# vLAR-group/unMORE

Measured on AMD Instinct MI355X. Metric: images/sec (train fwd+bwd) ObjectnessNet ViT-B/16 384x384, higher is better.
Workload: dtype bf16

## Files before the change

### unmore_amd/csrc/gemm_nt256p.hip

```cpp
#include "umr_common.h"
#include "gemm_epilogue.h"
#include <stdio.h>
#include <stdlib.h>
#include <type_traits>

namespace {

constexpr int BM2 = 256, BN2 = 256, BK2 = 64;
constexpr int ROWB2 = 128;
constexpr int TILE2 = 256 * ROWB2;
constexpr int BUF2 = 2 * TILE2;
constexpr int STG_OFF = 2 * BUF2;
constexpr int STG_BYTES = 32 * 256 * 4;
constexpr int LDS2P = STG_OFF + STG_BYTES;

typedef bf16_t T2;

__device__ __forceinline__ unsigned mul_dgelu_bf16x2(unsigned g, unsigned x) {
    const float lo = __builtin_bit_cast(float, g << 16) * dgelu_sel<bf16_t>(__builtin_bit_cast(float, x << 16));
    const float hi = __builtin_bit_cast(float, g & 0xFFFF0000u) * dgelu_sel<bf16_t>(__builtin_bit_cast(float, x & 0xFFFF0000u));
    typedef __attribute__((ext_vector_type(2))) __bf16 bf16x2;
    bf16x2 r;
    r[0] = (bf16_t)lo; r[1] = (bf16_t)hi;
    return __builtin_bit_cast(unsigned, r);
}

__device__ __forceinline__ unsigned add_bf16x2(unsigned x, unsigned y) {
    const float lo = __builtin_bit_cast(float, x << 16) + __builtin_bit_cast(float, y << 16);
    const float hi = __builtin_bit_cast(float, x & 0xFFFF0000u) + __builtin_bit_cast(float, y & 0xFFFF0000u);
    typedef __attribute__((ext_vector_type(2))) __bf16 bf16x2;
    bf16x2 r;
    r[0] = (bf16_t)lo; r[1] = (bf16_t)hi;
    return __builtin_bit_cast(unsigned, r);
}

__device__ __forceinline__ unsigned pos_mask_bf16x2(unsigned a) {
    typedef __attribute__((ext_vector_type(2))) short s16x2;
    const s16x2 one = {1, 1}, zero = {0, 0};
    s16x2 v = __builtin_bit_cast(s16x2, a);
    v = __builtin_elementwise_min(v, one);
    v = __builtin_elementwise_max(v, zero);
    v = zero - v;
    return __builtin_bit_cast(unsigned, v);
}

template <int CONV, int EPI, int AUXM, bool RED, bool X3 = false, bool P2 = true>
__global__ __launch_bounds__(512, 2) void gemm_nt256p_kernel(const umr_gemm_desc p, int tiles_n, int total_tiles, int stagger, int bm, int npairs = 6,
                                                             int kt_per_arg = 0) {
    const int sp = (X3 && kt_per_arg > 0) ? (int)blockIdx.y : 0;
    static_assert(X3 == (EPI == 5 || EPI == 6), "the plane-pair K loop and the f32 / plane epilogues (EPI 5, 6) go together");
    constexpr bool PH2 = P2;
    static_assert(CONV == 0 || P2, "the conv is instantiated in its two-phase form only");
    extern __shared__ __attribute__((aligned(16))) char smem[];
    constexpr int SZ = 2;
    constexpr unsigned OOB = 0x80000000u;
    const int tid = threadIdx.x, lane = tid & 63;
    const int w = __builtin_amdgcn_readfirstlane(tid >> 6);
    const bool ahead = (stagger != 0) && (w < 4);

    const int G = gridDim.x;
    const int pw = ((G & 7) == 0) ? (int)(blockIdx.x & 7) * (G >> 3) + (int)(blockIdx.x >> 3) : (int)blockIdx.x;
    if (pw >= total_tiles) return;
    const int n_my = (total_tiles - pw + G - 1) / G;

    const int lrow = lane >> 3, lchk = lane & 7;
    const int hw = (CONV != 0) ? p.Ho * p.Wo : 1;
    const int apix = X3 ? 3 * p.Cin : p.Cin;
    unsigned vo[4][2];
    int trow_a[2][2];
    unsigned a_tapmask[2][2];
    unsigned a_eff[2][2];
    int lds_row[4][2];
#pragma unroll
    for (int gi = 0; gi < 2; ++gi) {
#pragma unroll
        for (int i = 0; i < 2; ++i) {
            const int lr = (w * 2 + i) * 8 + lrow;
            {
                const int trow = (lr >> 6) * 128 + gi * 64 + (lr & 63);
                const int g = gi == 0 ? 0 : 3;
                lds_row[g][i] = (((w * 2 + i) * 8) >> 6) * 128 + gi * 64 + (((w * 2 + i) * 8) & 63);
                const int gch = lchk ^ ((trow >> 1) & 7);
                trow_a[gi][i] = trow;
                vo[g][i] = (CONV == 0) ? (unsigned)(((int64_t)trow * p.lda) * SZ + gch * 16)
                                       : (unsigned)((int64_t)trow * apix * SZ + gch * 16);
                a_eff[gi][i] = vo[g][i];
                a_tapmask[gi][i] = 0x1FFu;
            }
            {
                const int trow = (lr >> 5) * 64 + gi * 32 + (lr & 31);
                const int g = 1 + gi;
                lds_row[g][i] = (((w * 2 + i) * 8) >> 5) * 64 + gi * 32 + (((w * 2 + i) * 8) & 31);
                const int gch = lchk ^ ((trow >> 1) & 7);
                vo[g][i] = (unsigned)(((int64_t)trow * p.ldb) * SZ + gch * 16);
            }
        }
    }

    const int ktiles_per_tap = (CONV == 0) ? 0 : p.Cin / BK2;
    const int kt_total = (CONV == 0) ? p.K / BK2 : 9 * ktiles_per_tap;
    const int kb = sp * kt_per_arg;
    const int kt_mine = (X3 && kt_per_arg > 0) ? ((kt_total - kb < kt_per_arg) ? kt_total - kb : kt_per_arg) : kt_total;
    const int nt = kt_mine * (X3 ? npairs : 1);

    __amdgpu_buffer_rsrc_t rsA, rsB;
    int s_it = 0;
    int st_tile = 0, st_tap = 0, st_ci = 0, st_par = 0;
    int st_pp = 0, st_k = 0;
    unsigned soffA = 0, soffB = 0;
    auto clamp31 = [](int64_t v) -> int { return v > 0x7FFFFFFFll ? 0x7FFFFFFF : (v < 0 ? 0 : (int)v); };
    auto stage_setup = [&](int it) {
        const bool live = it < n_my;
        const int v = live ? it * G + pw : 0;
        const int tm = v / tiles_n, tn = v - tm * tiles_n;
        const int m0 = tm * bm, n0 = tn * BN2;
        st_tile = 0; st_pp = 0; st_k = kb;
        st_ci = (CONV == 0) ? 0 : kb / 9; st_tap = (CONV == 0) ? 0 : kb - st_ci * 9;
        rsB = __builtin_amdgcn_make_buffer_rsrc((void*)((const char*)p.B + (int64_t)n0 * p.ldb * SZ), 0,
                                                live ? clamp31((int64_t)(p.N - n0) * p.ldb * SZ) : 0, 0x00020000);
        if (CONV == 0) {
            rsA = __builtin_amdgcn_make_buffer_rsrc((void*)((const char*)p.A + (int64_t)m0 * p.lda * SZ), 0,
                                                    live ? clamp31((int64_t)((p.M - m0 < bm) ? (p.M - m0) : bm) * p.lda * SZ) : 0, 0x00020000);
        } else {
            rsA = __builtin_amdgcn_make_buffer_rsrc((void*)((const char*)p.A + ((int64_t)m0 - (p.W + 1)) * apix * SZ), 0,
                                                    live ? 0x7FFFFFFF : 0, 0x00020000);
#pragma unroll
            for (int gi = 0; gi < 2; ++gi)
#pragma unroll
                for (int i = 0; i < 2; ++i) {
                    const int m = m0 + trow_a[gi][i];
                    const int rem = m % hw;
                    const int oy = rem / p.Wo, ox = rem - oy * p.Wo;
                    unsigned mask = 0;
#pragma unroll
                    for (int tap = 0; tap < 9; ++tap) {
                        const int iy = oy - 1 + tap / 3, ix = ox - 1 + tap % 3;
                        if ((unsigned)iy < (unsigned)p.H && (unsigned)ix < (unsigned)p.W) mask |= 1u << tap;
                    }
                    a_tapmask[gi][i] = (live && m < p.M) ? mask : 0u;
                }
        }
    };
    auto stage_prep = [&]() {
        if (st_tile == nt) {
            ++s_it;
            stage_setup(s_it);
        }
        const int pa = X3 ? (((npairs == 6 ? 0x940 : 0x010) >> (2 * st_pp)) & 3) : 0;
        const int pb = X3 ? (((npairs == 6 ? 0x124 : 0x004) >> (2 * st_pp)) & 3) : 0;
        const bool next_k = !X3 || st_pp == npairs - 1;
        if (X3) st_pp = next_k ? 0 : st_pp + 1;
        if (CONV == 0) {
            const int kt = X3 ? st_k : st_tile;
            soffA = (unsigned)((kt * BK2 + pa * p.K) * SZ);
            soffB = (unsigned)((kt * BK2 + pb * p.K) * SZ);
            if (X3 && next_k) ++st_k;
        } else {
            const int c0 = st_ci * BK2;
            const int ky = st_tap / 3, kx = st_tap - ky * 3;
#pragma unroll
            for (int gi = 0; gi < 2; ++gi)
#pragma unroll
                for (int i = 0; i < 2; ++i)
                    a_eff[gi][i] = ((a_tapmask[gi][i] >> st_tap) & 1u) ? vo[gi == 0 ? 0 : 3][i] : OOB;
            soffA = (unsigned)(((ky * p.W + kx) * apix + pa * p.Cin + c0) * SZ);
            soffB = (unsigned)((pb * 9 * p.Cin + st_tap * p.Cin + c0) * SZ);
            if (next_k) { if (++st_tap == 9) { st_tap = 0; ++st_ci; } }
        }
    };
    auto stage_issue = [&](auto gtag, auto itag) {
        constexpr int Gp = decltype(gtag)::value, I = decltype(itag)::value;
        const unsigned v = (Gp == 0) ? a_eff[0][I] : (Gp == 3) ? a_eff[1][I] : vo[Gp][I];
        char* dst = smem + st_par * BUF2;
        if (Gp == 0 || Gp == 3) __builtin_amdgcn_raw_ptr_buffer_load_lds(rsA, UMR_LDS_PTR(dst + lds_row[Gp][I] * ROWB2), 16, v, soffA, 0, 0);
        else __builtin_amdgcn_raw_ptr_buffer_load_lds(rsB, UMR_LDS_PTR(dst + TILE2 + lds_row[Gp][I] * ROWB2), 16, v, soffB, 0, 0);
        if (Gp == 3 && I == 1) { ++st_tile; st_par ^= 1; }
    };
#define STAGE_DMA(Gp, I) stage_issue(std::integral_constant<int, Gp>{}, std::integral_constant<int, I>{})

    f32x4 acc[8][4];
    const int wr = w >> 2, wc = w & 3;
    const int dead_blocks = (CONV == 0 && wr == 1) ? ((BM2 - bm) >> 4) : 0;
    const int frow = lane & 15, fq = lane >> 4;
    int a_ad[2], b_ad[2];
#pragma unroll
    for (int ks = 0; ks < 2; ++ks) {
        const int q = ks * 4 + fq;
        const int sw = (frow >> 1) & 7;
        a_ad[ks] = (wr * 128 + frow) * ROWB2 + ((q ^ sw) << 4);
        b_ad[ks] = TILE2 + (wc * 64 + frow) * ROWB2 + ((q ^ sw) << 4);
    }
#define A_FRAG(ks, i) (*(const bf16x8*)(sbuf + a_ad[ks] + (i) * 16 * ROWB2))
#define B_FRAG(ks, i) (*(const bf16x8*)(sbuf + b_ad[ks] + (i) * 16 * ROWB2))

    bf16x8 fa[2][4], fb0[2][2], fb1[2][2];

#define PHASE_SYNC_N(N)                                            \
    asm volatile("s_waitcnt vmcnt(" #N ")" ::: "memory");          \
    __builtin_amdgcn_s_barrier();                                  \
    asm volatile("s_waitcnt lgkmcnt(0)" ::: "memory");             \
    __builtin_amdgcn_sched_barrier(0);
#define MFMA(ACC, BF, AF) ACC = __builtin_amdgcn_mfma_f32_16x16x32_bf16(BF, AF, ACC, 0, 0, 0)
    constexpr int PRIO_MODE = P2 ? 1 : 0;
#define QPRIO(x) if (PRIO_MODE == 0) __builtin_amdgcn_s_setprio(x);
#define QUADRANT_D(M0, N0, FB, DMA_A, DMA_B)                                                         \
    QPRIO(1)                                                                                        \
    MFMA(acc[M0 + 0][N0 + 0], FB[0][0], fa[0][0]); MFMA(acc[M0 + 0][N0 + 1], FB[0][1], fa[0][0]);   \
    MFMA(acc[M0 + 1][N0 + 0], FB[0][0], fa[0][1]); MFMA(acc[M0 + 1][N0 + 1], FB[0][1], fa[0][1]);   \
    __builtin_amdgcn_sched_barrier(0);                                                              \
    DMA_A;                                                                                          \
    __builtin_amdgcn_sched_barrier(0);                                                              \
    MFMA(acc[M0 + 2][N0 + 0], FB[0][0], fa[0][2]); MFMA(acc[M0 + 2][N0 + 1], FB[0][1], fa[0][2]);   \
    MFMA(acc[M0 + 3][N0 + 0], FB[0][0], fa[0][3]); MFMA(acc[M0 + 3][N0 + 1], FB[0][1], fa[0][3]);   \
    MFMA(acc[M0 + 0][N0 + 0], FB[1][0], fa[1][0]); MFMA(acc[M0 + 0][N0 + 1], FB[1][1], fa[1][0]);   \
    __builtin_amdgcn_sched_barrier(0);                                                              \
    DMA_B;                                                                                          \
    __builtin_amdgcn_sched_barrier(0);                                                              \
    MFMA(acc[M0 + 1][N0 + 0], FB[1][0], fa[1][1]); MFMA(acc[M0 + 1][N0 + 1], FB[1][1], fa[1][1]);   \
    MFMA(acc[M0 + 2][N0 + 0], FB[1][0], fa[1][2]); MFMA(acc[M0 + 2][N0 + 1], FB[1][1], fa[1][2]);   \
    MFMA(acc[M0 + 3][N0 + 0], FB[1][0], fa[1][3]); MFMA(acc[M0 + 3][N0 + 1], FB[1][1], fa[1][3]);   \
    QPRIO(0)
#define QUADRANT(M0, N0, FB, Gp) QUADRANT_D(M0, N0, FB, STAGE_DMA(Gp, 0), STAGE_DMA(Gp, 1))
#define QUADRANT_S(M0, N0, FB, Gp)                                                                  \
    QPRIO(1)                                                                                        \
    MFMA(acc[M0 + 0][N0 + 0], FB[0][0], fa[0][0]); MFMA(acc[M0 + 0][N0 + 1], FB[0][1], fa[0][0]);   \
    MFMA(acc[M0 + 1][N0 + 0], FB[0][0], fa[0][1]); MFMA(acc[M0 + 1][N0 + 1], FB[0][1], fa[0][1]);   \
    __builtin_amdgcn_sched_barrier(0);                                                              \
    STAGE_DMA(Gp, 0);                                                                               \
    __builtin_amdgcn_sched_barrier(0);                                                              \
    MFMA(acc[M0 + 0][N0 + 0], FB[1][0], fa[1][0]); MFMA(acc[M0 + 0][N0 + 1], FB[1][1], fa[1][0]);   \
    MFMA(acc[M0 + 1][N0 + 0], FB[1][0], fa[1][1]); MFMA(acc[M0 + 1][N0 + 1], FB[1][1], fa[1][1]);   \
    __builtin_amdgcn_sched_barrier(0);                                                              \
    STAGE_DMA(Gp, 1);                                                                               \
    __builtin_amdgcn_sched_barrier(0);                                                              \
    QPRIO(0)
#define QUADRANT_HI(N0, FB, Gp)                                                  \
    if (dead_blocks == 0) { QUADRANT(4, N0, FB, Gp) }                            \
    else if (dead_blocks == 2) { QUADRANT_S(4, N0, FB, Gp) }                     \
    else { STAGE_DMA(Gp, 0); STAGE_DMA(Gp, 1); }

#define QUADRANT_SD(M0, N0, FB, DMA_A, DMA_B)                                                        \
    QPRIO(1)                                                                                        \
    MFMA(acc[M0 + 0][N0 + 0], FB[0][0], fa[0][0]); MFMA(acc[M0 + 0][N0 + 1], FB[0][1], fa[0][0]);   \
    MFMA(acc[M0 + 1][N0 + 0], FB[0][0], fa[0][1]); MFMA(acc[M0 + 1][N0 + 1], FB[0][1], fa[0][1]);   \
    __builtin_amdgcn_sched_barrier(0);                                                              \
    DMA_A;                                                                                          \
    __builtin_amdgcn_sched_barrier(0);                                                              \
    MFMA(acc[M0 + 0][N0 + 0], FB[1][0], fa[1][0]); MFMA(acc[M0 + 0][N0 + 1], FB[1][1], fa[1][0]);   \
    MFMA(acc[M0 + 1][N0 + 0], FB[1][0], fa[1][1]); MFMA(acc[M0 + 1][N0 + 1], FB[1][1], fa[1][1]);   \
    __builtin_amdgcn_sched_barrier(0);                                                              \
    DMA_B;                                                                                          \
    __builtin_amdgcn_sched_barrier(0);                                                              \
    QPRIO(0)
#define QUADRANT_HID(N0, FB, DMA_A, DMA_B)                                       \
    if (dead_blocks == 0) { QUADRANT_D(4, N0, FB, DMA_A, DMA_B) }                \
    else if (dead_blocks == 2) { QUADRANT_SD(4, N0, FB, DMA_A, DMA_B) }          \
    else { DMA_A; DMA_B; }

#define PHASE_SYNC() PHASE_SYNC_N(6)
    auto tile_body2 = [&](const char* sbuf) {
#pragma unroll
        for (int ks = 0; ks < 2; ++ks) {
#pragma unroll
            for (int i = 0; i < 2; ++i) fb0[ks][i] = B_FRAG(ks, i);
#pragma unroll
            for (int i = 0; i < 4; ++i) fa[ks][i] = A_FRAG(ks, i);
#pragma unroll
            for (int i = 0; i < 2; ++i) fb1[ks][i] = B_FRAG(ks, 2 + i);
        }
        PHASE_SYNC_N(6);
        QUADRANT_D(0, 0, fb0, STAGE_DMA(3, 0), STAGE_DMA(3, 1))
        QUADRANT_D(0, 2, fb1, (void)0, (void)0)
        stage_prep();
#pragma unroll
        for (int ks = 0; ks < 2; ++ks)
#pragma unroll
            for (int i = 0; i < 4; ++i) fa[ks][i] = A_FRAG(ks, 4 + i);
        PHASE_SYNC_N(2);
        QUADRANT_HID(2, fb1, STAGE_DMA(0, 0); STAGE_DMA(0, 1), STAGE_DMA(1, 0); STAGE_DMA(1, 1))
        QUADRANT_HID(0, fb0, STAGE_DMA(2, 0), STAGE_DMA(2, 1))
    };
    auto tile_body = [&](const char* sbuf) {
        if (PH2) { tile_body2(sbuf); return; }
#pragma unroll
        for (int ks = 0; ks < 2; ++ks) {
#pragma unroll
            for (int i = 0; i < 2; ++i) fb0[ks][i] = B_FRAG(ks, i);
#pragma unroll
            for (int i = 0; i < 4; ++i) fa[ks][i] = A_FRAG(ks, i);
        }
        PHASE_SYNC();
        QUADRANT(0, 0, fb0, 2)
#pragma unroll
        for (int ks = 0; ks < 2; ++ks)
#pragma unroll
            for (int i = 0; i < 2; ++i) fb1[ks][i] = B_FRAG(ks, 2 + i);
        PHASE_SYNC();
        QUADRANT(0, 2, fb1, 3)
        stage_prep();
#pragma unroll
        for (int ks = 0; ks < 2; ++ks)
#pragma unroll
            for (int i = 0; i < 4; ++i) fa[ks][i] = A_FRAG(ks, 4 + i);
        PHASE_SYNC();
        QUADRANT_HI(2, fb1, 0)
        PHASE_SYNC();
        QUADRANT_HI(0, fb0, 1)
    };

#define READ_WAIT()                                                \
    asm volatile("s_waitcnt lgkmcnt(0)" ::: "memory");             \
    __builtin_amdgcn_sched_barrier(0);
#define END_SYNC_N(N)                                              \
    asm volatile("s_waitcnt vmcnt(" #N ")" ::: "memory");          \
    __builtin_amdgcn_s_barrier();                                  \
    __builtin_amdgcn_sched_barrier(0);
    auto tile_body2_ahead = [&](const char* sbuf) {
        stage_prep();
#pragma unroll
        for (int ks = 0; ks < 2; ++ks) {
#pragma unroll
            for (int i = 0; i < 2; ++i) fb0[ks][i] = B_FRAG(ks, i);
#pragma unroll
            for (int i = 0; i < 4; ++i) fa[ks][i] = A_FRAG(ks, i);
#pragma unroll
            for (int i = 0; i < 2; ++i) fb1[ks][i] = B_FRAG(ks, 2 + i);
        }
        READ_WAIT();
        QUADRANT_D(0, 0, fb0, STAGE_DMA(0, 0); STAGE_DMA(0, 1), STAGE_DMA(1, 0); STAGE_DMA(1, 1))
        QUADRANT_D(0, 2, fb1, STAGE_DMA(2, 0), STAGE_DMA(2, 1))
        END_SYNC_N(6);
#pragma unroll
        for (int ks = 0; ks < 2; ++ks)
#pragma unroll
            for (int i = 0; i < 4; ++i) fa[ks][i] = A_FRAG(ks, 4 + i);
        READ_WAIT();
        QUADRANT_HID(2, fb1, STAGE_DMA(3, 0), STAGE_DMA(3, 1))
        QUADRANT_HID(0, fb0, (void)0, (void)0)
        END_SYNC_N(2);
    };
    auto tile_body4_ahead = [&](const char* sbuf) {
#pragma unroll
        for (int ks = 0; ks < 2; ++ks) {
#pragma unroll
            for (int i = 0; i < 2; ++i) fb0[ks][i] = B_FRAG(ks, i);
#pragma unroll
            for (int i = 0; i < 4; ++i) fa[ks][i] = A_FRAG(ks, i);
        }
        READ_WAIT();
        QUADRANT(0, 0, fb0, 1)
        END_SYNC_N(6);
#pragma unroll
        for (int ks = 0; ks < 2; ++ks)
#pragma unroll
            for (int i = 0; i < 2; ++i) fb1[ks][i] = B_FRAG(ks, 2 + i);
        READ_WAIT();
        QUADRANT(0, 2, fb1, 2)
        END_SYNC_N(6);
#pragma unroll
        for (int ks = 0; ks < 2; ++ks)
#pragma unroll
            for (int i = 0; i < 4; ++i) fa[ks][i] = A_FRAG(ks, 4 + i);
        READ_WAIT();
        QUADRANT(4, 2, fb1, 3)
        END_SYNC_N(6);
        stage_prep();
        QUADRANT(4, 0, fb0, 0)
        END_SYNC_N(6);
    };

    if (PRIO_MODE == 1 && w >= 4) __builtin_amdgcn_s_setprio(1);
    stage_setup(0);
    stage_prep();
    STAGE_DMA(0, 0); STAGE_DMA(0, 1); STAGE_DMA(1, 0); STAGE_DMA(1, 1);
    STAGE_DMA(2, 0); STAGE_DMA(2, 1); STAGE_DMA(3, 0); STAGE_DMA(3, 1);
    if (ahead) {
        if (PH2) {
            asm volatile("s_waitcnt vmcnt(2)" ::: "memory");
        } else {
            stage_prep();
            STAGE_DMA(0, 0); STAGE_DMA(0, 1);
            asm volatile("s_waitcnt vmcnt(6)" ::: "memory");
        }
    } else {
        stage_prep();
        STAGE_DMA(0, 0); STAGE_DMA(0, 1); STAGE_DMA(1, 0); STAGE_DMA(1, 1);
        if (PH2) { STAGE_DMA(2, 0); STAGE_DMA(2, 1); }
        asm volatile("s_waitcnt vmcnt(8)" ::: "memory");
    }
    __builtin_amdgcn_s_barrier();

    const int er = lane >> 3, ec = lane & 7;
    const unsigned co_lane = ((unsigned)((w >> 2) * 128 + er) * (unsigned)p.ldc + (unsigned)((w & 3) * 64 + ec * 8)) * 2u;
    const unsigned ax_lane = ((unsigned)((w >> 2) * 128 + er) * (unsigned)p.ldaux + (unsigned)((w & 3) * 64 + ec * 8)) * 2u;
    constexpr int WST_BYTES = 2048;
    constexpr int RW_OFF = 8 * WST_BYTES;
    float* stg = (float*)(smem + STG_OFF);
    auto stage_rows = [&](auto mtag) {
        constexpr int MT = decltype(mtag)::value;
        const int lr = wr * 16 + frow;
#pragma unroll
        for (int ntl = 0; ntl < 4; ++ntl) {
            const int ch = (wc * 16 + ntl * 4 + fq) ^ frow;
            *(f32x4*)(stg + lr * 256 + ch * 4) = acc[MT][ntl];
        }
    };
    int c_par = 0;
    constexpr bool BIAS_INIT = (EPI == 3 || EPI == 4 || EPI == 5 || EPI == 6);
    f32x4 bqn[4];
    auto fetch_bias = [&](int it_) {
        const int v_ = it_ * G + pw;
        const int tn_ = v_ - (v_ / tiles_n) * tiles_n;
#pragma unroll
        for (int ntl = 0; ntl < 4; ++ntl) {
            const int n = tn_ * BN2 + wc * 64 + ntl * 16 + fq * 4;
            bqn[ntl] = f32x4{0.f, 0.f, 0.f, 0.f};
            if ((p.flags & UMR_EPI_BIAS) && it_ < n_my && n < p.N) bqn[ntl] = *(const f32x4*)(p.bias + n);
        }
    };
    if (BIAS_INIT) fetch_bias(0);
#pragma unroll 1
    for (int it = 0; it < n_my; ++it) {
#pragma unroll
        for (int i = 0; i < 8; ++i)
#pragma unroll
            for (int j = 0; j < 4; ++j) acc[i][j] = BIAS_INIT ? bqn[j] : f32x4{0.f, 0.f, 0.f, 0.f};
        if (RED && w < 2) {
            const int v_ = it * G + pw;
            const int n0_ = (v_ - (v_ / tiles_n) * tiles_n) * BN2;
            const __amdgpu_buffer_rsrc_t rsW = __builtin_amdgcn_make_buffer_rsrc(
                (void*)(p.red_w + (int64_t)w * p.N + n0_), 0, (w < p.red_c) ? clamp31((int64_t)(p.N - n0_) * 4) : 0, 0x00020000);
            const int rw_off = (EPI == 3) ? RW_OFF + (it & 1) * 2048 : 0;
            __builtin_amdgcn_raw_ptr_buffer_load_lds(rsW, UMR_LDS_PTR(smem + STG_OFF + rw_off + w * 1024), 16, (unsigned)(lane * 16), 0, 0, 0);
        }
        if (ahead) {
#pragma unroll 1
            for (int t = 0; t < nt; ++t) {
                if (PH2) tile_body2_ahead(smem + c_par * BUF2); else tile_body4_ahead(smem + c_par * BUF2);
                c_par ^= 1;
            }
        } else {
#pragma unroll 1
            for (int t = 0; t < nt; ++t) {
                tile_body(smem + c_par * BUF2);
                c_par ^= 1;
            }
        }
        const int v = it * G + pw;
        const int tm = v / tiles_n, tn = v - tm * tiles_n;
        const int m0 = tm * bm, n0 = tn * BN2;
        const int m_end = (p.M - m0 < bm) ? p.M : m0 + bm;
        if (EPI == 3) {
            fetch_bias(it + 1);
            typedef __attribute__((ext_vector_type(2))) short s16x2;
            typedef __attribute__((ext_vector_type(2))) unsigned u32x2;
            const short relu_lo = (p.act == UMR_ACT_RELU) ? (short)0 : (short)-32768;
            const s16x2 relu16 = {relu_lo, relu_lo};
            auto pack4 = [&](const f32x4& v) -> u32x2 {
                unsigned lo, hi;
                asm("v_cvt_pk_bf16_f32 %0, %1, %2" : "=v"(lo) : "v"(v[0]), "v"(v[1]));
                asm("v_cvt_pk_bf16_f32 %0, %1, %2" : "=v"(hi) : "v"(v[2]), "v"(v[3]));
                s16x2 a = __builtin_bit_cast(s16x2, lo), b = __builtin_bit_cast(s16x2, hi);
                if (AUXM == 0) {
                    a = __builtin_elementwise_max(a, relu16);
                    b = __builtin_elementwise_max(b, relu16);
                }
                return u32x2{__builtin_bit_cast(unsigned, a), __builtin_bit_cast(unsigned, b)};
            };
            bf16x8 rwh[2], rwl[2];
            float* ro_lane = nullptr;
            if (RED) {
#pragma unroll
                for (int pr = 0; pr < 2; ++pr) {
                    f32x4 a = {0.f, 0.f, 0.f, 0.f}, b = {0.f, 0.f, 0.f, 0.f};
                    if (frow < 2) {
                        const char* rwp = smem + STG_OFF + RW_OFF + (it & 1) * 2048 + frow * 1024;
                        a = *(const f32x4*)(rwp + (wc * 64 + (2 * pr) * 16 + fq * 4) * 4);
                        b = *(const f32x4*)(rwp + (wc * 64 + (2 * pr + 1) * 16 + fq * 4) * 4);
                    }
#pragma unroll
                    for (int e = 0; e < 8; ++e) {
                        const float x = e < 4 ? a[e] : b[e - 4];
                        const bf16_t hi = (bf16_t)x;
                        rwh[pr][e] = hi;
                        rwl[pr][e] = (bf16_t)(x - (float)hi);
                    }
                }
                if (fq == 0 && n0 + wc * 64 < p.N)
                    ro_lane = p.red_out + ((int64_t)(tn * 4 + wc) * p.M + (m0 + wr * 128 + frow)) * p.red_c;
            }
            auto row_reduce2 = [&](const bf16x8& a01, const bf16x8& a23, const bf16x8& b01, const bf16x8& b23, int mt_) {
                const f32x4 z = {0.f, 0.f, 0.f, 0.f};
                f32x4 ra = __builtin_amdgcn_mfma_f32_16x16x32_bf16(rwh[0], a01, z, 0, 0, 0);
                f32x4 rb = __builtin_amdgcn_mfma_f32_16x16x32_bf16(rwh[0], b01, z, 0, 0, 0);
                ra = __builtin_amdgcn_mfma_f32_16x16x32_bf16(rwl[0], a01, ra, 0, 0, 0);
                rb = __builtin_amdgcn_mfma_f32_16x16x32_bf16(rwl[0], b01, rb, 0, 0, 0);
                ra = __builtin_amdgcn_mfma_f32_16x16x32_bf16(rwh[1], a23, ra, 0, 0, 0);
                rb = __builtin_amdgcn_mfma_f32_16x16x32_bf16(rwh[1], b23, rb, 0, 0, 0);
                ra = __builtin_amdgcn_mfma_f32_16x16x32_bf16(rwl[1], a23, ra, 0, 0, 0);
                rb = __builtin_amdgcn_mfma_f32_16x16x32_bf16(rwl[1], b23, rb, 0, 0, 0);
                const int m = m0 + wr * 128 + mt_ * 16 + frow;
                if (ro_lane != nullptr) {
                    float* ro = ro_lane + (int64_t)(mt_ * 16) * p.red_c;
                    if (p.red_c == 2) {
                        if (m < m_end) *(f32x2*)ro = f32x2{ra[0], ra[1]};
                        if (m + 16 < m_end) *(f32x2*)(ro + 32) = f32x2{rb[0], rb[1]};
                    } else {
                        if (m < m_end) ro[0] = ra[0];
                        if (m + 16 < m_end) ro[16] = rb[0];
                    }
                }
            };
            const bool col_live = n0 + wc * 64 + ec * 8 < p.N;
            const __amdgpu_buffer_rsrc_t rsC = __builtin_amdgcn_make_buffer_rsrc(
                (void*)((T2*)p.C + (int64_t)m0 * p.ldc + n0), 0, p.no_store ? 0 : clamp31((int64_t)(m_end - m0) * p.ldc * 2), 0x00020000);
            const unsigned co_vo = col_live ? co_lane : OOB;
            __amdgpu_buffer_rsrc_t rsX = rsC;
            unsigned ax_vo = OOB;
            if (AUXM != 0) {
                rsX = __builtin_amdgcn_make_buffer_rsrc((void*)((T2*)p.aux + (int64_t)m0 * p.ldaux + n0), 0,
                                                        clamp31((int64_t)(m_end - m0) * p.ldaux * 2), 0x00020000);
                ax_vo = col_live ? ax_lane : OOB;
            }
            u32x4 axc[4][2];
            auto load_auxc = [&](auto btag) {
                constexpr int MB = decltype(btag)::value;
                if (MB < 8 && AUXM != 0) {
#pragma unroll
                    for (int k = 0; k < 2; ++k)
                        axc[MB & 3][k] = __builtin_amdgcn_raw_buffer_load_b128(rsX, ax_vo + (unsigned)((MB * 16 + k * 8) * p.ldaux * 2), 0, 0);
                }
            };
            load_auxc(std::integral_constant<int, 0>{});
            load_auxc(std::integral_constant<int, 1>{});
            char* wst = smem + STG_OFF + w * WST_BYTES;
            const int wsw = (frow >> 1) & 7;
            char* wst_w = wst + frow * 128 + (fq & 1) * 8;
            const char* wst_r0 = wst + er * 128 + ((ec ^ ((er >> 1) & 7)) << 4);
            const char* wst_r1 = wst + (er + 8) * 128 + ((ec ^ (((er >> 1) + 4) & 7)) << 4);
            auto blocks2 = [&](auto btag) {
                constexpr int MB = decltype(btag)::value;
                load_auxc(std::integral_constant<int, MB + 2>{});
                load_auxc(std::integral_constant<int, MB + 3>{});
                u32x2 pk[2][4];
#pragma unroll
                for (int mh = 0; mh < 2; ++mh)
#pragma unroll
                    for (int ntl = 0; ntl < 4; ++ntl) pk[mh][ntl] = pack4(acc[MB + mh][ntl]);
                if (RED) {
                    bf16x8 tq[2][2];
#pragma unroll
                    for (int mh = 0; mh < 2; ++mh)
#pragma unroll
                        for (int h = 0; h < 2; ++h)
                            tq[mh][h] = __builtin_bit_cast(bf16x8, u32x4{pk[mh][2 * h][0], pk[mh][2 * h][1], pk[mh][2 * h + 1][0], pk[mh][2 * h + 1][1]});
                    row_reduce2(tq[0][0], tq[0][1], tq[1][0], tq[1][1], MB);
                }
#pragma unroll
                for (int mh = 0; mh < 2; ++mh) {
#pragma unroll
                    for (int ntl = 0; ntl < 4; ++ntl) *(u32x2*)(wst_w + (((ntl * 2 + (fq >> 1)) ^ wsw) << 4)) = pk[mh][ntl];
                    asm volatile("" ::: "memory");
                    u32x4 o[2];
                    o[0] = *(const u32x4*)wst_r0;
                    o[1] = *(const u32x4*)wst_r1;
                    asm volatile("" ::: "memory");
#pragma unroll
                    for (int k = 0; k < 2; ++k) {
                        if (AUXM == 2) {
                            const u32x4 a = axc[(MB + mh) & 3][k];
#pragma unroll
                            for (int e = 0; e < 4; ++e) o[k][e] &= pos_mask_bf16x2(a[e]);
                        }
                        if (AUXM == 1) {
                            const u32x4 a = axc[(MB + mh) & 3][k];
#pragma unroll
                            for (int e = 0; e < 4; ++e) o[k][e] = add_bf16x2(o[k][e], a[e]);
                        }
                        const unsigned so = (unsigned)(((MB + mh) * 16 + k * 8) * p.ldc * 2);
                        __builtin_amdgcn_raw_buffer_store_b128(o[k], rsC, co_vo + so, 0, 0);
                    }
                }
            };
            if (RED && p.no_store) {
#pragma unroll
                for (int mt = 0; mt < 8; mt += 2) {
                    bf16x8 tq[2][2];
#pragma unroll
                    for (int mh = 0; mh < 2; ++mh)
#pragma unroll
                        for (int ntl = 0; ntl < 4; ++ntl) {
                            const bf16x4 t = __builtin_bit_cast(bf16x4, pack4(acc[mt + mh][ntl]));
#pragma unroll
                            for (int e = 0; e < 4; ++e) tq[mh][ntl >> 1][(ntl & 1) * 4 + e] = t[e];
                        }
                    row_reduce2(tq[0][0], tq[0][1], tq[1][0], tq[1][1], mt);
                }
            } else {
                blocks2(std::integral_constant<int, 0>{}); blocks2(std::integral_constant<int, 2>{});
                blocks2(std::integral_constant<int, 4>{}); blocks2(std::integral_constant<int, 6>{});
            }
        } else if (EPI == 4) {
            fetch_bias(it + 1);
            constexpr bool dgelu = (AUXM == 2);
            const bool two_out = !dgelu && p.c2_mode == 2;
            typedef __attribute__((ext_vector_type(2))) unsigned u32x2;
            const bool col_live = n0 + wc * 64 + ec * 8 < p.N;
            const __amdgpu_buffer_rsrc_t rsC = __builtin_amdgcn_make_buffer_rsrc(
                (void*)((T2*)p.C + (int64_t)m0 * p.ldc + n0), 0, clamp31((int64_t)(m_end - m0) * p.ldc * 2), 0x00020000);
            const unsigned co_vo = col_live ? co_lane : OOB;
            __amdgpu_buffer_rsrc_t rsC2 = rsC, rsX = rsC;
            unsigned c2_vo = OOB, ax_vo = OOB;
            if (two_out) {
                rsC2 = __builtin_amdgcn_make_buffer_rsrc((void*)((T2*)p.C2 + (int64_t)m0 * p.ldc2 + n0), 0,
                                                         clamp31((int64_t)(m_end - m0) * p.ldc2 * 2), 0x00020000);
                c2_vo = col_live ? ((unsigned)(wr * 128 + er) * (unsigned)p.ldc2 + (unsigned)(wc * 64 + ec * 8)) * 2u : OOB;
            }
            if (dgelu) {
                rsX = __builtin_amdgcn_make_buffer_rsrc((void*)((T2*)p.aux + (int64_t)m0 * p.ldaux + n0), 0,
                                                        clamp31((int64_t)(m_end - m0) * p.ldaux * 2), 0x00020000);
                ax_vo = col_live ? ax_lane : OOB;
            }
            u32x4 axc[4][2];
            auto load_auxc = [&](auto btag) {
                constexpr int MB = decltype(btag)::value;
                if (MB < 8 && dgelu) {
#pragma unroll
                    for (int k = 0; k < 2; ++k)
                        axc[MB & 3][k] = __builtin_amdgcn_raw_buffer_load_b128(rsX, ax_vo + (unsigned)((MB * 16 + k * 8) * p.ldaux * 2), 0, 0);
                }
            };
            load_auxc(std::integral_constant<int, 0>{});
            load_auxc(std::integral_constant<int, 1>{});
            char* wst = smem + STG_OFF + w * WST_BYTES;
            const int wsw = (frow >> 1) & 7;
            char* wst_w = wst + frow * 128 + (fq & 1) * 8;
            const char* wst_r0 = wst + er * 128 + ((ec ^ ((er >> 1) & 7)) << 4);
            const char* wst_r1 = wst + (er + 8) * 128 + ((ec ^ (((er >> 1) + 4) & 7)) << 4);
            auto pack4g = [&](const f32x4& v) -> u32x2 {
                unsigned lo, hi;
                asm("v_cvt_pk_bf16_f32 %0, %1, %2" : "=v"(lo) : "v"(v[0]), "v"(v[1]));
                asm("v_cvt_pk_bf16_f32 %0, %1, %2" : "=v"(hi) : "v"(v[2]), "v"(v[3]));
                return u32x2{lo, hi};
            };
            auto block4 = [&](auto btag) {
                constexpr int MB = decltype(btag)::value;
                load_auxc(std::integral_constant<int, MB + 2>{});
                if (two_out) {
#pragma unroll
                    for (int ntl = 0; ntl < 4; ++ntl) *(u32x2*)(wst_w + (((ntl * 2 + (fq >> 1)) ^ wsw) << 4)) = pack4g(acc[MB][ntl]);
                    asm volatile("" ::: "memory");
                    const u32x4 o0 = *(const u32x4*)wst_r0, o1 = *(const u32x4*)wst_r1;
                    asm volatile("" ::: "memory");
                    __builtin_amdgcn_raw_buffer_store_b128(o0, rsC2, c2_vo + (unsigned)((MB * 16) * p.ldc2 * 2), 0, 0);
                    __builtin_amdgcn_raw_buffer_store_b128(o1, rsC2, c2_vo + (unsigned)((MB * 16 + 8) * p.ldc2 * 2), 0, 0);
                }
#pragma unroll
                for (int ntl = 0; ntl < 4; ++ntl) {
                    f32x4 v = acc[MB][ntl];
                    if (!dgelu) {
#pragma unroll
                        for (int e = 0; e < 4; ++e) v[e] = gelu_sel<T2>(v[e]);
                    }
                    *(u32x2*)(wst_w + (((ntl * 2 + (fq >> 1)) ^ wsw) << 4)) = pack4g(v);
                }
                asm volatile("" ::: "memory");
                u32x4 o[2];
                o[0] = *(const u32x4*)wst_r0;
                o[1] = *(const u32x4*)wst_r1;
                asm volatile("" ::: "memory");
#pragma unroll
                for (int k = 0; k < 2; ++k) {
                    if (dgelu) {
                        const u32x4 a = axc[MB & 3][k];
#pragma unroll
                        for (int e = 0; e < 4; ++e) o[k][e] = mul_dgelu_bf16x2(o[k][e], a[e]);
                    }
                    __builtin_amdgcn_raw_buffer_store_b128(o[k], rsC, co_vo + (unsigned)((MB * 16 + k * 8) * p.ldc * 2), 0, 0);
                }
            };
            block4(std::integral_constant<int, 0>{}); block4(std::integral_constant<int, 1>{});
            block4(std::integral_constant<int, 2>{}); block4(std::integral_constant<int, 3>{});
            block4(std::integral_constant<int, 4>{}); block4(std::integral_constant<int, 5>{});
            block4(std::integral_constant<int, 6>{}); block4(std::integral_constant<int, 7>{});
        } else if (EPI == 5 || EPI == 6) {
            fetch_bias(it + 1);
            const float relu_floor = (p.act == UMR_ACT_RELU) ? 0.f : -INFINITY;
            const bool planes = (p.flags & UMR_EPI_OUT_X3) != 0;
            const bool maskf = (p.flags & UMR_EPI_MASK_RELU) != 0;
            const bool maskp = (p.flags & UMR_EPI_AUX_X3) != 0;
            if (RED) {
                f32x4 rw[2][4];
#pragma unroll
                for (int c = 0; c < 2; ++c)
#pragma unroll
                    for (int ntl = 0; ntl < 4; ++ntl)
                        rw[c][ntl] = *(const f32x4*)(smem + STG_OFF + c * 1024 + (wc * 64 + ntl * 16 + fq * 4) * 4);
#pragma unroll
                for (int mt = 0; mt < 8; ++mt) {
                    float rs0 = 0.f, rs1 = 0.f;
#pragma unroll
                    for (int ntl = 0; ntl < 4; ++ntl) {
                        const f32x4 v = acc[mt][ntl];
#pragma unroll
                        for (int e = 0; e < 4; ++e) {
                            const float t = fmaxf(v[e], relu_floor);
                            rs0 += t * rw[0][ntl][e];
                            rs1 += t * rw[1][ntl][e];
                        }
                    }
                    rs0 += __shfl_xor(rs0, 16, 64); rs0 += __shfl_xor(rs0, 32, 64);
                    rs1 += __shfl_xor(rs1, 16, 64); rs1 += __shfl_xor(rs1, 32, 64);
                    const int m = m0 + wr * 128 + mt * 16 + frow;
                    if (fq == 0 && m < m_end && n0 + wc * 64 < p.N) {
                        float* ro = p.red_out + ((int64_t)(tn * 4 + wc) * p.M + m) * p.red_c;
                        ro[0] = rs0;
                        if (p.red_c == 2) ro[1] = rs1;
                    }
                }
            } else {
#pragma unroll 1
            for (int mt = 0; mt < 8; ++mt) {
                if (mt > 0) __syncthreads();
                switch (mt) {
                    case 0: stage_rows(std::integral_constant<int, 0>{}); break;
                    case 1: stage_rows(std::integral_constant<int, 1>{}); break;
                    case 2: stage_rows(std::integral_constant<int, 2>{}); break;
                    case 3: stage_rows(std::integral_constant<int, 3>{}); break;
                    case 4: stage_rows(std::integral_constant<int, 4>{}); break;
                    case 5: stage_rows(std::integral_constant<int, 5>{}); break;
                    case 6: stage_rows(std::integral_constant<int, 6>{}); break;
                    default: stage_rows(std::integral_constant<int, 7>{}); break;
                }
                __syncthreads();
                constexpr int UNROLL_J = (EPI == 6) ? 1 : 2;
#pragma clang loop unroll_count(UNROLL_J)
                for (int j = 0; j < 2; ++j) {
                    const int lr = (tid >> 5) + j * 16, cg = tid & 31;
                    const int m = m0 + (lr >> 4) * 128 + mt * 16 + (lr & 15), n = n0 + cg * 8;
                    if (m >= m_end || n >= p.N) continue;
                    const int sw = lr & 15;
                    f32x4 v0 = *(const f32x4*)(stg + lr * 256 + (((2 * cg) ^ sw) << 2));
                    f32x4 v1 = *(const f32x4*)(stg + lr * 256 + (((2 * cg + 1) ^ sw) << 2));
                    if constexpr (EPI == 6) {
                        x3_epilogue_store8<false>(p, m, n, v0, v1);
                    } else {
#pragma unroll
                        for (int e = 0; e < 4; ++e) { v0[e] = fmaxf(v0[e], relu_floor); v1[e] = fmaxf(v1[e], relu_floor); }
                        if (maskf) {
                            f32x4 a0, a1;
                            if (maskp) {
                                const bf16x8 h = *(const bf16x8*)((const T2*)p.aux + (int64_t)m * p.ldaux + n);
                                a0 = f32x4{(float)h[0], (float)h[1], (float)h[2], (float)h[3]};
                                a1 = f32x4{(float)h[4], (float)h[5], (float)h[6], (float)h[7]};
                            } else {
                                const float* ap = (const float*)p.aux + (int64_t)m * p.ldaux + n;
                                a0 = *(const f32x4*)ap; a1 = *(const f32x4*)(ap + 4);
                            }
#pragma unroll
                            for (int e = 0; e < 4; ++e) { v0[e] = a0[e] > 0.f ? v0[e] : 0.f; v1[e] = a1[e] > 0.f ? v1[e] : 0.f; }
                        }
                        const int64_t mo = m + (int64_t)sp * p.M;
                        if (planes) x3_planes_store8((T2*)p.C + mo * p.ldc + n, p.N, v0, v1);
                        else { float* cp = (float*)p.C + mo * p.ldc + n; *(f32x4*)cp = v0; *(f32x4*)(cp + 4) = v1; }
                    }
                }
            }
            }
        } else {
            const bool vec_ok = ((p.N & 7) == 0) && ((p.ldc & 7) == 0) && ((p.ldc2 & 7) == 0) && ((p.ldaux & 7) == 0) &&
                                ((p.ldaux2 & 7) == 0);
#pragma unroll 1
            for (int mt = 0; mt < 8; ++mt) {
                if (mt > 0) __syncthreads();
                switch (mt) {
                    case 0: stage_rows(std::integral_constant<int, 0>{}); break;
                    case 1: stage_rows(std::integral_constant<int, 1>{}); break;
                    case 2: stage_rows(std::integral_constant<int, 2>{}); break;
                    case 3: stage_rows(std::integral_constant<int, 3>{}); break;
                    case 4: stage_rows(std::integral_constant<int, 4>{}); break;
                    case 5: stage_rows(std::integral_constant<int, 5>{}); break;
                    case 6: stage_rows(std::integral_constant<int, 6>{}); break;
                    default: stage_rows(std::integral_constant<int, 7>{}); break;
                }
                __syncthreads();
#pragma unroll 1
                for (int j = 0; j < 2; ++j) {
                    const int lr = (tid >> 5) + j * 16, cg = tid & 31;
                    const int m = m0 + (lr >> 4) * 128 + mt * 16 + (lr & 15), n = n0 + cg * 8;
                    if (m >= m_end || n >= p.N) continue;
                    const int sw = lr & 15;
                    const f32x4 v0 = *(const f32x4*)(stg + lr * 256 + (((2 * cg) ^ sw) << 2));
                    const f32x4 v1 = *(const f32x4*)(stg + lr * 256 + (((2 * cg + 1) ^ sw) << 2));
                    if (vec_ok) {
                        epilogue_store8<T2>(p, m, n, v0, v1);
                    } else {
                        epilogue_store<T2>(p, m, n, v0);
                        if (n + 4 < p.N) epilogue_store<T2>(p, m, n + 4, v1);
                    }
                }
            }
        }
        __syncthreads();
    }
    asm volatile("s_waitcnt vmcnt(0)" ::: "memory");
#undef QUADRANT
#undef QUADRANT_S
#undef QUADRANT_HI
#undef QUADRANT_HID
#undef QUADRANT_SD
#undef QUADRANT_D
#undef MFMA
#undef PHASE_SYNC
#undef PHASE_SYNC_N
#undef STAGE_DMA
#undef READ_WAIT
#undef END_SYNC_N
#undef A_FRAG
#undef B_FRAG
}

__global__ __launch_bounds__(256) void x3_splitk_finish_kernel(const umr_gemm_desc p, const float* __restrict__ slabs, int ksplit, int64_t slab_stride) {
    const int n8 = p.N >> 3;
    const int64_t total = (int64_t)p.M * n8;
    for (int64_t idx = (int64_t)blockIdx.x * blockDim.x + threadIdx.x; idx < total; idx += (int64_t)gridDim.x * blockDim.x) {
        const int m = (int)(idx / n8);
        const int n = (int)(idx - (int64_t)m * n8) * 8;
        const float* q = slabs + (int64_t)m * p.N + n;
        f32x4 v0 = *(const f32x4*)q, v1 = *(const f32x4*)(q + 4);
        for (int s_ = 1; s_ < ksplit; ++s_) {
            const float* qs = q + s_ * slab_stride;
            v0 += *(const f32x4*)qs; v1 += *(const f32x4*)(qs + 4);
        }
        x3_epilogue_store8<true>(p, m, n, v0, v1);
    }
}

int num_cus() {
    static const int n = [] {
        int dev = 0;
        hipDeviceProp_t prop;
        return (hipGetDevice(&dev) == hipSuccess && hipGetDeviceProperties(&prop, dev) == hipSuccess && prop.multiProcessorCount > 0)
                   ? prop.multiProcessorCount : 256;
    }();
    return n;
}

}

bool umr_nt256p_fast_epilogue(const umr_gemm_desc* d) {
    const bool vec_ok = ((d->N & 7) == 0) && ((d->ldc & 7) == 0) && ((d->ldaux & 7) == 0);
    const bool mask = (d->flags & UMR_EPI_MASK_RELU) != 0, add = (d->flags & UMR_EPI_ADD_AUX) != 0;
    return vec_ok && d->c2_mode == 0 && d->c_rows_in <= 0 && d->aux_mod <= 0 &&
           !(d->flags & (UMR_EPI_ROWBIAS | UMR_EPI_ADD_AUX2 | UMR_EPI_OUT_F32 | UMR_EPI_MASK_DGELU)) && !(mask && add) &&
           (d->act == UMR_ACT_NONE || (d->act == UMR_ACT_RELU && !mask && !add));
}
bool umr_nt256p_plain_epilogue(const umr_gemm_desc* d) {
    return umr_nt256p_fast_epilogue(d) && (!d->red_w || (d->conv == 0 && !(d->flags & (UMR_EPI_ADD_AUX | UMR_EPI_MASK_RELU))));
}

static bool umr_nt256p_gelu_epilogue(const umr_gemm_desc* d) {
    const bool vec_ok = ((d->N & 7) == 0) && ((d->ldc & 7) == 0) && ((d->ldaux & 7) == 0) && ((d->ldc2 & 7) == 0);
    const bool dg = (d->flags & UMR_EPI_MASK_DGELU) != 0;
    return vec_ok && (d->c2_mode == 0 || (d->c2_mode == 2 && !dg)) && d->c_rows_in <= 0 && d->aux_mod <= 0 && !d->red_w && !d->no_store &&
           !(d->flags & (UMR_EPI_ROWBIAS | UMR_EPI_ADD_AUX2 | UMR_EPI_OUT_F32 | UMR_EPI_MASK_RELU | UMR_EPI_ADD_AUX)) &&
           ((d->act == UMR_ACT_GELU && !dg) || (d->act == UMR_ACT_NONE && dg));
}

static void x3_plan(const umr_gemm_desc* d, int cus, int npairs, int64_t ws_bytes, int* bm_out, int* ks_out) {
    const int tiles_n = (d->N + BN2 - 1) / BN2;
    const int kt = d->conv == 0 ? d->K / BK2 : 9 * (d->Cin / BK2);
    const int bm_env = umr_opt_or(UMR_OPT_NT256_BM, 0);
    const int64_t slab = (int64_t)d->M * d->N * 4;
    int best_ks = 1, best_bm = BM2;
    double best_cost = 1e300;
    for (int bm = BM2; bm >= (d->conv == 0 ? 192 : BM2); bm -= 32) {
        if (d->conv == 0 && (bm_env == 256 || bm_env == 224 || bm_env == 192) && bm != bm_env) continue;
        const int64_t tiles = (int64_t)((d->M + bm - 1) / bm) * tiles_n;
        for (int ks = 1; ks <= 32 && ks * 2 <= kt + 1; ++ks) {
            if (d->red_w && ks > 1) break;
            if (ks > 1 && ((int64_t)ks * slab > ws_bytes)) break;
            const int per = (kt + ks - 1) / ks;
            if ((kt + per - 1) / per != ks) continue;
            const int64_t rounds = (tiles * ks + cus - 1) / cus;
            const double cost = (double)rounds * (per * npairs * (bm / 256.0) + 8.0) + (ks > 1 ? 8.0 + (double)ks * slab / 4.5e6 : 0.0);
            if (cost < best_cost * (ks > best_ks ? 0.90 : 0.98)) { best_cost = cost; best_ks = ks; best_bm = bm; }
        }
    }
    *bm_out = best_bm;
    *ks_out = best_ks;
}

extern "C" int64_t umr_gemm_nt_x3_workspace(const umr_gemm_desc* d) {
    if (d == nullptr || d->dtype != UMR_BF16X3 || d->M <= 0 || d->N <= 0 || d->K <= 0) return 0;
    int bm, ks;
    x3_plan(d, num_cus(), umr_f32_mode_now() == UMR_F32_X3_FAST ? 3 : 6, (int64_t)1 << 40, &bm, &ks);
    return ks > 1 ? (int64_t)ks * d->M * d->N * 4 : 0;
// ... 139 lines not shown
```

Measured before the change: 350.3.

## Overlap epilogue stores with next tile and stage bias through LDS

For the bias/store epilogues (EPI 3 and 4), bias is loaded asynchronously into LDS by buffer_load_lds and read back with ds_read, replacing per-thread global loads. The end-of-tile __syncthreads is dropped for these epilogues. The first K tile of the next output tile uses a looser vmcnt wait that accounts for outstanding epilogue stores, so stores can overlap the next tile's loads and MFMAs. Reduction stores now go through buffer stores with range-checked resources instead of guarded pointer writes, and lane ids are recomputed to relieve register pressure. The hand-tuned vmcnt counts and the removed barrier risk races or stalls if the counts are off.

After: 348.5. Within noise of the previous version (-0.5%).

```diff
diff --git a/unmore_amd/csrc/gemm_nt256p.hip b/unmore_amd/csrc/gemm_nt256p.hip
--- a/unmore_amd/csrc/gemm_nt256p.hip
+++ b/unmore_amd/csrc/gemm_nt256p.hip
@@ -42,6 +42,12 @@
     v = __builtin_elementwise_max(v, zero);
     v = zero - v;
     return __builtin_bit_cast(unsigned, v);
+}
+
+__device__ __forceinline__ int lane_id_fresh() {
+    int l;
+    asm volatile("v_mbcnt_lo_u32_b32 %0, -1, 0\n\tv_mbcnt_hi_u32_b32 %0, -1, %0" : "=v"(l));
+    return l;
 }
 
 template <int CONV, int EPI, int AUXM, bool RED, bool X3 = false, bool P2 = true>
@@ -57,6 +63,8 @@
     const int tid = threadIdx.x, lane = tid & 63;
     const int w = __builtin_amdgcn_readfirstlane(tid >> 6);
     const bool ahead = (stagger != 0) && (w < 4);
+    constexpr bool STORE_AWARE = (EPI == 3 || EPI == 4);
+    bool kt_first = false;
 
     const int G = gridDim.x;
     const int pw = ((G & 7) == 0) ? (int)(blockIdx.x & 7) * (G >> 3) + (int)(blockIdx.x >> 3) : (int)blockIdx.x;
@@ -200,6 +208,14 @@
     __builtin_amdgcn_s_barrier();                                  \
     asm volatile("s_waitcnt lgkmcnt(0)" ::: "memory");             \
     __builtin_amdgcn_sched_barrier(0);
+#define TILE_WAIT(N, NS)                                                       \
+    if (kt_first) asm volatile("s_waitcnt vmcnt(" #NS ")" ::: "memory");       \
+    else asm volatile("s_waitcnt vmcnt(" #N ")" ::: "memory");
+#define PHASE_SYNC_F(N, NS)                                        \
+    TILE_WAIT(N, NS)                                               \
+    __builtin_amdgcn_s_barrier();                                  \
+    asm volatile("s_waitcnt lgkmcnt(0)" ::: "memory");             \
+    __builtin_amdgcn_sched_barrier(0);
 #define MFMA(ACC, BF, AF) ACC = __builtin_amdgcn_mfma_f32_16x16x32_bf16(BF, AF, ACC, 0, 0, 0)
     constexpr int PRIO_MODE = P2 ? 1 : 0;
 #define QPRIO(x) if (PRIO_MODE == 0) __builtin_amdgcn_s_setprio(x);
@@ -257,7 +273,7 @@
     else if (dead_blocks == 2) { QUADRANT_SD(4, N0, FB, DMA_A, DMA_B) }          \
     else { DMA_A; DMA_B; }
 
-#define PHASE_SYNC() PHASE_SYNC_N(6)
+#define PHASE_SYNC() PHASE_SYNC_F(6, 22)
     auto tile_body2 = [&](const char* sbuf) {
 #pragma unroll
         for (int ks = 0; ks < 2; ++ks) {
@@ -268,7 +284,7 @@
 #pragma unroll
             for (int i = 0; i < 2; ++i) fb1[ks][i] = B_FRAG(ks, 2 + i);
         }
-        PHASE_SYNC_N(6);
+        PHASE_SYNC_F(6, 22);
         QUADRANT_D(0, 0, fb0, STAGE_DMA(3, 0), STAGE_DMA(3, 1))
         QUADRANT_D(0, 2, fb1, (void)0, (void)0)
         stage_prep();
@@ -276,7 +292,7 @@
         for (int ks = 0; ks < 2; ++ks)
 #pragma unroll
             for (int i = 0; i < 4; ++i) fa[ks][i] = A_FRAG(ks, 4 + i);
-        PHASE_SYNC_N(2);
+        PHASE_SYNC_F(2, 18);
         QUADRANT_HID(2, fb1, STAGE_DMA(0, 0); STAGE_DMA(0, 1), STAGE_DMA(1, 0); STAGE_DMA(1, 1))
         QUADRANT_HID(0, fb0, STAGE_DMA(2, 0), STAGE_DMA(2, 1))
     };
@@ -315,6 +331,10 @@
     asm volatile("s_waitcnt vmcnt(" #N ")" ::: "memory");          \
     __builtin_amdgcn_s_barrier();                                  \
     __builtin_amdgcn_sched_barrier(0);
+#define END_SYNC_F(N, NS)                                          \
+    TILE_WAIT(N, NS)                                               \
+    __builtin_amdgcn_s_barrier();                                  \
+    __builtin_amdgcn_sched_barrier(0);
     auto tile_body2_ahead = [&](const char* sbuf) {
         stage_prep();
 #pragma unroll
@@ -329,7 +349,7 @@
         READ_WAIT();
         QUADRANT_D(0, 0, fb0, STAGE_DMA(0, 0); STAGE_DMA(0, 1), STAGE_DMA(1, 0); STAGE_DMA(1, 1))
         QUADRANT_D(0, 2, fb1, STAGE_DMA(2, 0), STAGE_DMA(2, 1))
-        END_SYNC_N(6);
+        END_SYNC_F(6, 22);
 #pragma unroll
         for (int ks = 0; ks < 2; ++ks)
 #pragma unroll
@@ -349,21 +369,21 @@
         }
         READ_WAIT();
         QUADRANT(0, 0, fb0, 1)
-        END_SYNC_N(6);
+        END_SYNC_F(6, 22);
 #pragma unroll
         for (int ks = 0; ks < 2; ++ks)
 #pragma unroll
             for (int i = 0; i < 2; ++i) fb1[ks][i] = B_FRAG(ks, 2 + i);
         READ_WAIT();
         QUADRANT(0, 2, fb1, 2)
-        END_SYNC_N(6);
+        END_SYNC_F(6, 22);
 #pragma unroll
         for (int ks = 0; ks < 2; ++ks)
 #pragma unroll
             for (int i = 0; i < 4; ++i) fa[ks][i] = A_FRAG(ks, 4 + i);
         READ_WAIT();
         QUADRANT(4, 2, fb1, 3)
-        END_SYNC_N(6);
+        END_SYNC_F(6, 22);
         stage_prep();
         QUADRANT(4, 0, fb0, 0)
         END_SYNC_N(6);
@@ -390,9 +410,6 @@
     }
     __builtin_amdgcn_s_barrier();
 
-    const int er = lane >> 3, ec = lane & 7;
-    const unsigned co_lane = ((unsigned)((w >> 2) * 128 + er) * (unsigned)p.ldc + (unsigned)((w & 3) * 64 + ec * 8)) * 2u;
-    const unsigned ax_lane = ((unsigned)((w >> 2) * 128 + er) * (unsigned)p.ldaux + (unsigned)((w & 3) * 64 + ec * 8)) * 2u;
     constexpr int WST_BYTES = 2048;
     constexpr int RW_OFF = 8 * WST_BYTES;
     float* stg = (float*)(smem + STG_OFF);
@@ -408,7 +425,7 @@
     int c_par = 0;
     constexpr bool BIAS_INIT = (EPI == 3 || EPI == 4 || EPI == 5 || EPI == 6);
     f32x4 bqn[4];
-    auto fetch_bias = [&](int it_) {
+    auto fetch_bias = [&](int it_, int fq) {
         const int v_ = it_ * G + pw;
         const int tn_ = v_ - (v_ / tiles_n) * tiles_n;
 #pragma unroll
@@ -418,9 +435,38 @@
             if ((p.flags & UMR_EPI_BIAS) && it_ < n_my && n < p.N) bqn[ntl] = *(const f32x4*)(p.bias + n);
         }
     };
-    if (BIAS_INIT) fetch_bias(0);
+    constexpr bool BIAS_LDS = (EPI == 3 || EPI == 4);
+    constexpr int BIAS_OFF = RW_OFF + 2 * 2048;
+    static_assert(BIAS_OFF + 8 * 256 <= STG_BYTES, "bias blocks fit the staging region");
+    auto issue_bias = [&](int it_) {
+        const int v_ = it_ * G + pw;
+        const int n_ = (v_ - (v_ / tiles_n) * tiles_n) * BN2 + wc * 64;
+        const bool on = (p.flags & UMR_EPI_BIAS) && it_ < n_my && n_ < p.N;
+        const __amdgpu_buffer_rsrc_t rsb = __builtin_amdgcn_make_buffer_rsrc((void*)(p.bias + (on ? n_ : 0)), 0,
+                                                                             on ? clamp31((int64_t)(p.N - n_) * 4) : 0, 0x00020000);
+        __builtin_amdgcn_raw_ptr_buffer_load_lds(rsb, UMR_LDS_PTR(smem + STG_OFF + BIAS_OFF + w * 256), 4, (unsigned)(lane_id_fresh() * 4), 0, 0, 0);
+    };
+    auto read_bias = [&](bool stores) {
+        const unsigned ad = (unsigned)(uintptr_t)UMR_LDS_PTR(smem + STG_OFF + BIAS_OFF + w * 256) + (unsigned)((lane_id_fresh() >> 4) * 16);
+        if (stores) asm volatile("s_waitcnt vmcnt(18)" ::: "memory");
+        else asm volatile("s_waitcnt vmcnt(2)" ::: "memory");
+        asm volatile("ds_read_b128 %0, %4\n\t"
+                     "ds_read_b128 %1, %4 offset:64\n\t"
+                     "ds_read_b128 %2, %4 offset:128\n\t"
+                     "ds_read_b128 %3, %4 offset:192\n\t"
+                     "s_waitcnt lgkmcnt(0)"
+                     : "=&v"(bqn[0]), "=&v"(bqn[1]), "=&v"(bqn[2]), "=&v"(bqn[3])
+                     : "v"(ad)
+                     : "memory");
+    };
+    if (BIAS_LDS) issue_bias(0);
+    else if (BIAS_INIT) fetch_bias(0, fq);
 #pragma unroll 1
     for (int it = 0; it < n_my; ++it) {
+        if (BIAS_LDS) {
+            read_bias(!(RED && p.no_store));
+            issue_bias(it + 1);
+        }
 #pragma unroll
         for (int i = 0; i < 8; ++i)
 #pragma unroll
@@ -431,17 +477,19 @@
             const __amdgpu_buffer_rsrc_t rsW = __builtin_amdgcn_make_buffer_rsrc(
                 (void*)(p.red_w + (int64_t)w * p.N + n0_), 0, (w < p.red_c) ? clamp31((int64_t)(p.N - n0_) * 4) : 0, 0x00020000);
             const int rw_off = (EPI == 3) ? RW_OFF + (it & 1) * 2048 : 0;
-            __builtin_amdgcn_raw_ptr_buffer_load_lds(rsW, UMR_LDS_PTR(smem + STG_OFF + rw_off + w * 1024), 16, (unsigned)(lane * 16), 0, 0, 0);
+            __builtin_amdgcn_raw_ptr_buffer_load_lds(rsW, UMR_LDS_PTR(smem + STG_OFF + rw_off + w * 1024), 16, (unsigned)(lane_id_fresh() * 16), 0, 0, 0);
         }
         if (ahead) {
 #pragma unroll 1
             for (int t = 0; t < nt; ++t) {
+                kt_first = STORE_AWARE && t == 0 && it > 0 && !(RED && p.no_store);
                 if (PH2) tile_body2_ahead(smem + c_par * BUF2); else tile_body4_ahead(smem + c_par * BUF2);
                 c_par ^= 1;
             }
         } else {
 #pragma unroll 1
             for (int t = 0; t < nt; ++t) {
+                kt_first = STORE_AWARE && t == 0 && it > 0 && !(RED && p.no_store);
                 tile_body(smem + c_par * BUF2);
                 c_par ^= 1;
             }
@@ -451,7 +499,10 @@
         const int m0 = tm * bm, n0 = tn * BN2;
         const int m_end = (p.M - m0 < bm) ? p.M : m0 + bm;
         if (EPI == 3) {
-            fetch_bias(it + 1);
+            const int lane_e = lane_id_fresh();
+            const int frow = lane_e & 15, fq = lane_e >> 4, er = lane_e >> 3, ec = lane_e & 7;
+            const unsigned co_lane = ((unsigned)(wr * 128 + er) * (unsigned)p.ldc + (unsigned)(wc * 64 + ec * 8)) * 2u;
+            const unsigned ax_lane = ((unsigned)(wr * 128 + er) * (unsigned)p.ldaux + (unsigned)(wc * 64 + ec * 8)) * 2u;
             typedef __attribute__((ext_vector_type(2))) short s16x2;
             typedef __attribute__((ext_vector_type(2))) unsigned u32x2;
             const short relu_lo = (p.act == UMR_ACT_RELU) ? (short)0 : (short)-32768;
@@ -468,7 +519,8 @@
                 return u32x2{__builtin_bit_cast(unsigned, a), __builtin_bit_cast(unsigned, b)};
             };
             bf16x8 rwh[2], rwl[2];
-            float* ro_lane = nullptr;
+            unsigned ro_vo = OOB;
+            __amdgpu_buffer_rsrc_t rsR = __builtin_amdgcn_make_buffer_rsrc((void*)p.red_out, 0, 0, 0x00020000);
             if (RED) {
 #pragma unroll
                 for (int pr = 0; pr < 2; ++pr) {
@@ -486,8 +538,9 @@
                         rwl[pr][e] = (bf16_t)(x - (float)hi);
                     }
                 }
-                if (fq == 0 && n0 + wc * 64 < p.N)
-                    ro_lane = p.red_out + ((int64_t)(tn * 4 + wc) * p.M + (m0 + wr * 128 + frow)) * p.red_c;
+                rsR = __builtin_amdgcn_make_buffer_rsrc((void*)(p.red_out + ((int64_t)(tn * 4 + wc) * p.M + m0) * p.red_c), 0,
+                                                        (n0 + wc * 64 < p.N) ? clamp31((int64_t)(m_end - m0) * p.red_c * 4) : 0, 0x00020000);
+                if (fq == 0) ro_vo = (unsigned)((wr * 128 + frow) * p.red_c * 4);
             }
             auto row_reduce2 = [&](const bf16x8& a01, const bf16x8& a23, const bf16x8& b01, const bf16x8& b23, int mt_) {
                 const f32x4 z = {0.f, 0.f, 0.f, 0.f};
@@ -499,16 +552,14 @@
                 rb = __builtin_amdgcn_mfma_f32_16x16x32_bf16(rwh[1], b23, rb, 0, 0, 0);
                 ra = __builtin_amdgcn_mfma_f32_16x16x32_bf16(rwl[1], a23, ra, 0, 0, 0);
                 rb = __builtin_amdgcn_mfma_f32_16x16x32_bf16(rwl[1], b23, rb, 0, 0, 0);
-                const int m = m0 + wr * 128 + mt_ * 16 + frow;
-                if (ro_lane != nullptr) {
-                    float* ro = ro_lane + (int64_t)(mt_ * 16) * p.red_c;
-                    if (p.red_c == 2) {
-                        if (m < m_end) *(f32x2*)ro = f32x2{ra[0], ra[1]};
-                        if (m + 16 < m_end) *(f32x2*)(ro + 32) = f32x2{rb[0], rb[1]};
-                    } else {
-                        if (m < m_end) ro[0] = ra[0];
-                        if (m + 16 < m_end) ro[16] = rb[0];
-                    }
+                typedef __attribute__((ext_vector_type(2))) unsigned u32x2;
+                const unsigned so = ro_vo + (unsigned)(mt_ * 16 * p.red_c * 4);
+                if (p.red_c == 2) {
+                    __builtin_amdgcn_raw_buffer_store_b64(__builtin_bit_cast(u32x2, f32x2{ra[0], ra[1]}), rsR, so, 0, 0);
+                    __builtin_amdgcn_raw_buffer_store_b64(__builtin_bit_cast(u32x2, f32x2{rb[0], rb[1]}), rsR, so + 128u, 0, 0);
+                } else {
+                    __builtin_amdgcn_raw_buffer_store_b32(__builtin_bit_cast(unsigned, ra[0]), rsR, so, 0, 0);
+                    __builtin_amdgcn_raw_buffer_store_b32(__builtin_bit_cast(unsigned, rb[0]), rsR, so + 64u, 0, 0);
                 }
             };
             const bool col_live = n0 + wc * 64 + ec * 8 < p.N;
@@ -601,7 +652,10 @@
                 blocks2(std::integral_constant<int, 4>{}); blocks2(std::integral_constant<int, 6>{});
             }
         } else if (EPI == 4) {
-            fetch_bias(it + 1);
+            const int lane_e = lane_id_fresh();
+            const int frow = lane_e & 15, fq = lane_e >> 4, er = lane_e >> 3, ec = lane_e & 7;
+            const unsigned co_lane = ((unsigned)(wr * 128 + er) * (unsigned)p.ldc + (unsigned)(wc * 64 + ec * 8)) * 2u;
+            const unsigned ax_lane = ((unsigned)(wr * 128 + er) * (unsigned)p.ldaux + (unsigned)(wc * 64 + ec * 8)) * 2u;
             constexpr bool dgelu = (AUXM == 2);
             const bool two_out = !dgelu && p.c2_mode == 2;
             typedef __attribute__((ext_vector_type(2))) unsigned u32x2;
@@ -684,7 +738,7 @@
             block4(std::integral_constant<int, 4>{}); block4(std::integral_constant<int, 5>{});
             block4(std::integral_constant<int, 6>{}); block4(std::integral_constant<int, 7>{});
         } else if (EPI == 5 || EPI == 6) {
-            fetch_bias(it + 1);
+            fetch_bias(it + 1, fq);
             const float relu_floor = (p.act == UMR_ACT_RELU) ? 0.f : -INFINITY;
             const bool planes = (p.flags & UMR_EPI_OUT_X3) != 0;
             const bool maskf = (p.flags & UMR_EPI_MASK_RELU) != 0;
@@ -801,7 +855,7 @@
                 }
             }
         }
-        __syncthreads();
+        if (EPI != 3 && EPI != 4) __syncthreads();
     }
     asm volatile("s_waitcnt vmcnt(0)" ::: "memory");
 #undef QUADRANT
@@ -813,6 +867,9 @@
 #undef MFMA
 #undef PHASE_SYNC
 #undef PHASE_SYNC_N
+#undef PHASE_SYNC_F
+#undef END_SYNC_F
+#undef TILE_WAIT
 #undef STAGE_DMA
 #undef READ_WAIT
 #undef END_SYNC_N
```
